# deryrahman/image-caption-emotion-indonesia

Hardware: AMD Instinct MI355X
Metric: images/sec (train step) + NLL loss match, batch=64 ResNet152+FactoredLSTM-512 (higher is better)
Workload: dtype f32 (trunk: operands as 2 f16 pieces each, 3 MFMA products per multiply, f32 accumulate; decoder: large products as 3 bf16 pieces per operand, 6 MFMA products per multiply, the rest f32 MFMA; the persistent LSTM kernel the trunk's split-f16 scheme)

## Files before the change

image-caption-emotion-indonesia_amd/csrc/fused_block.hip:

```cpp
#include <cstdlib>
#include <type_traits>

#include "common.h"
#include "mfma_core.h"
#include "split_f16.h"
#include "kernels.h"

namespace capnet {
namespace {

__host__ __device__ constexpr int fb_kslot(int g, int j) { return 16 * (j >> 2) + 4 * g + (j & 3); }


__global__ __launch_bounds__(256) void fb_pack_kernel(const float* __restrict__ w, unsigned* __restrict__ img, int C, int MID,
                                                      int role, int wide) {
  const int ew = f16x3_weight_shift(img[1]);
  if (blockIdx.x == 0 && threadIdx.x == 0) { img[0] = (unsigned)ew; img[2] = (unsigned)wide; }
  const float ws = ldexpf(1.f, ew);
  const long cells = (long)C * MID / 8 * 2;
  for (long i = (long)blockIdx.x * blockDim.x + threadIdx.x; i < cells; i += (long)gridDim.x * blockDim.x) {
    long r = i;
    const int lane = (int)(r & 63); r >>= 6;
    const int plane = (int)(r & 1); r >>= 1;
    const float* src;
// ... 30 lines not shown
      }
    }
    unsigned out[4];
#pragma unroll
    for (int q = 0; q < 4; ++q) {
      const float x0 = src[koff[2 * q]] * ws, x1 = src[koff[2 * q + 1]] * ws;
      _Float16 h0, l0, h1, l1;
      split1(x0, h0, l0);
      split1(x1, h1, l1);
      const h2 p = plane == 0 ? h2{h0, h1} : h2{l0, l1};
      out[q] = __builtin_bit_cast(unsigned, p);
    }
    unsigned* dst = img + kF16x3HdrWords + i * 4;
    dst[0] = out[0]; dst[1] = out[1]; dst[2] = out[2]; dst[3] = out[3];
  }
  if (role == 0) {
    float* cp = reinterpret_cast<float*>(img + kF16x3HdrWords + (long)C * MID);
    for (long i = (long)blockIdx.x * blockDim.x + threadIdx.x; i < (long)C * MID; i += (long)gridDim.x * blockDim.x) {
      const int c = (int)(i / MID), k = (int)(i - (long)c * MID);
      cp[((long)(c >> 4) * MID + k) * 16 + (c & 15)] = w[i];
    }
  }
}

static inline int fb_gram_rows(int K) { return K == 64 ? 512 : 256; }

struct GArgs {
  const float* y2; const float* s2; const float* t2;
  float* gp;
  float* cs;
  int M, K, in_exp, slices, pairs, slice_rows;
};

template <int K>
__global__ __launch_bounds__(256) void fb_gram_kernel(const GArgs g) {
  constexpr int NBLK = K / 64, NPAIR = NBLK * (NBLK + 1) / 2;
  constexpr int SR = K == 64 ? 128 : 64, NRG = SR / 8;
  constexpr int NCQ = K / 4, NIT = NCQ * NRG / 256;
  constexpr int kPlane = NRG * K * 16;
  static_assert(NIT >= 1 && NCQ * NRG == NIT * 256, "staging items");
  __shared__ __attribute__((aligned(16))) unsigned char lds[2 * kPlane];
  const int tid = threadIdx.x, lane = tid & 63, wave = tid >> 6;
  const int wm = wave >> 1, wn = wave & 1, li = lane & 31, lh = lane >> 5;
  const int slice = blockIdx.x, row0 = slice * g.slice_rows;
  const int rows = min(g.slice_rows, g.M - row0);
  const int nst = (rows + SR - 1) / SR;
  const float iscale = ldexpf(1.f, g.in_exp);
  const int chq = tid % NCQ, rgb = tid / NCQ;
  const f32x4 sc = *reinterpret_cast<const f32x4*>(g.s2 + 4 * chq), sh = *reinterpret_cast<const f32x4*>(g.t2 + 4 * chq);
  f32x4 colsum = {0.f, 0.f, 0.f, 0.f};
  f32x16 acc[NPAIR];
#pragma unroll
  for (int p = 0; p < NPAIR; ++p)
#pragma unroll
    for (int r = 0; r < 16; ++r) acc[p][r] = 0.f;
  f32x4 v[NIT][8];
  auto fetch = [&](int st) __attribute__((always_inline)) {
#pragma unroll
    for (int q = 0; q < NIT; ++q)
#pragma unroll
      for (int e = 0; e < 8; ++e) {
        const int m = row0 + st * SR + (rgb + q * (256 / NCQ)) * 8 + e;
        v[q][e] = *reinterpret_cast<const f32x4*>(g.y2 + (long)min(m, g.M - 1) * K + 4 * chq);
      }
  };
  auto stage = [&](int st) __attribute__((always_inline)) {
#pragma unroll
    for (int q = 0; q < NIT; ++q) {
      const int rg = rgb + q * (256 / NCQ);
      f32x4 x[8];
#pragma unroll
      for (int e = 0; e < 8; ++e) {
        const bool ok = row0 + st * SR + rg * 8 + e < row0 + rows;
#pragma unroll
        for (int c = 0; c < 4; ++c) {
          const float t = fmaxf(fmaf(v[q][e][c], sc[c], sh[c]), 0.f) * iscale;
          x[e][c] = ok ? t : 0.f;
          colsum[c] += x[e][c];
        }
      }
#pragma unroll
      for (int c = 0; c < 4; ++c) {
        const f32x4 a = {x[0][c], x[1][c], x[2][c], x[3][c]}, b = {x[4][c], x[5][c], x[6][c], x[7][c]};
        h4 ha, la, hb, lb;
        split4(a, ha, la);
        split4(b, hb, lb);
        unsigned char* d = lds + (rg * K + 4 * chq + c) * 16;
        *reinterpret_cast<h8*>(d) = cat8(ha, hb);
        *reinterpret_cast<h8*>(d + kPlane) = cat8(la, lb);
      }
    }
  };
  auto mma = [&]() __attribute__((always_inline)) {
#pragma unroll 2
    for (int k = 0; k < NRG / 2; ++k) {
      const unsigned char* base = lds + ((2 * k + lh) * K + li) * 16;
      h8 ah[NBLK], al[NBLK], bh[NBLK], bl[NBLK];
#pragma unroll
      for (int b = 0; b < NBLK; ++b) {
        ah[b] = *reinterpret_cast<const h8*>(base + (b * 64 + wm * 32) * 16);
        al[b] = *reinterpret_cast<const h8*>(base + (b * 64 + wm * 32) * 16 + kPlane);
        bh[b] = *reinterpret_cast<const h8*>(base + (b * 64 + wn * 32) * 16);
        bl[b] = *reinterpret_cast<const h8*>(base + (b * 64 + wn * 32) * 16 + kPlane);
      }
      int p = 0;
#pragma unroll
      for (int bi = 0; bi < NBLK; ++bi)
#pragma unroll
        for (int bj = bi; bj < NBLK; ++bj, ++p) {
          acc[p] = __builtin_amdgcn_mfma_f32_32x32x16_f16(al[bi], bh[bj], acc[p], 0, 0, 0);
          acc[p] = __builtin_amdgcn_mfma_f32_32x32x16_f16(ah[bi], bl[bj], acc[p], 0, 0, 0);
          acc[p] = __builtin_amdgcn_mfma_f32_32x32x16_f16(ah[bi], bh[bj], acc[p], 0, 0, 0);
        }
    }
  };
  fetch(0);
  for (int st = 0; st < nst; ++st) {
    stage(st);
    __syncthreads();
    fetch(st + 1 < nst ? st + 1 : st);
    mma();
    __syncthreads();
  }
  const float osc = ldexpf(1.f, -2 * g.in_exp);
#pragma unroll
  for (int p = 0; p < NPAIR; ++p) {
#pragma unroll
    for (int r = 0; r < 16; ++r) {
      const int m = wm * 32 + (r & 3) + 8 * (r >> 2) + 4 * lh;
      g.gp[(((long)p * 64 + m) * g.slices + slice) * 64 + wn * 32 + li] = acc[p][r] * osc;
    }
  }
  f32x4* cs_sh = reinterpret_cast<f32x4*>(lds);
  cs_sh[tid] = colsum;
  __syncthreads();
  if (tid < NCQ) {
    f32x4 t = cs_sh[tid];
#pragma unroll
    for (int q = 1; q < 256 / NCQ; ++q) t += cs_sh[q * NCQ + tid];
    *reinterpret_cast<f32x4*>(g.cs + (long)slice * K + 4 * tid) = t * ldexpf(1.f, -g.in_exp);
  }
}

__global__ __launch_bounds__(256) void fb_gram_reduce_kernel(const float* __restrict__ gp, const float* __restrict__ cs, float* __restrict__ G,
                                                             float* __restrict__ mu, int K, int slices, int pairs) {
  __shared__ double sh[8][32][4];
  const int it = threadIdx.x & 31, part = threadIdx.x >> 5;
  const int item_wgs = pairs * 32;
  if ((int)blockIdx.x < item_wgs) {
    const int item = blockIdx.x * 32 + it;
    const int n4 = item & 15, m = (item >> 4) & 63, pair = item >> 10;
    const float* p = gp + ((long)(pair * 64 + m) * slices) * 64 + 4 * n4;
    double s[4] = {0.0, 0.0, 0.0, 0.0};
    for (int s0 = part; s0 < slices; s0 += 64) {
      f32x4 v[8];
#pragma unroll
      for (int u = 0; u < 8; ++u) {
        const int sl = s0 + 8 * u;
        v[u] = *reinterpret_cast<const f32x4*>(p + (long)(sl < slices ? sl : part) * 64);
      }
#pragma unroll
      for (int u = 0; u < 8; ++u)
#pragma unroll
        for (int i = 0; i < 4; ++i) s[i] += (s0 + 8 * u < slices) ? (double)v[u][i] : 0.0;
    }
#pragma unroll
    for (int i = 0; i < 4; ++i) sh[part][it][i] = s[i];
    __syncthreads();
    if (part == 0) {
#pragma unroll
      for (int q = 1; q < 8; ++q)
#pragma unroll
        for (int i = 0; i < 4; ++i) s[i] += sh[q][it][i];
// ... 631 lines not shown
bool fused_block_shape_ok(long M, int MID) {
  return (MID == 64 || MID == 128 || MID == 256) && M > 0 && M < (1l << 24) && M * 4 * MID * 4 < (1l << 32);
}

size_t fused_block_weight_words(int C, int MID, int role) {
  return (size_t)kF16x3HdrWords + (size_t)C * MID * (role == 0 ? 2 : 1);
}

static bool fb_wide(int MID) {
  const char* e = getenv("CAPNET_FB_WIDE");
  if (e && (e[0] == '0' || e[0] == '1')) return e[0] == '1';
  (void)MID;
  return false;
}

int fused_block_pack(const float* w, unsigned* img, int C, int MID, int role, hipStream_t stream) {
  CAPNET_REQUIRE(w && img && aligned16(img) && C == 4 * MID && (MID == 64 || MID == 128 || MID == 256) && (role == 0 || role == 1),
                 "fused_block_pack: bad argument (C=%d MID=%d role=%d)", C, MID, role);
  const long n = (long)C * MID;
  const int rh = f16x3_pack_header(w, img, n, stream);
  if (rh) return rh;
  hipLaunchKernelGGL(fb_pack_kernel, dim3((int)(cdiv(n / 4, 256) > 2048 ? 2048 : cdiv(n / 4, 256))), dim3(256), 0, stream, w, img, C, MID, role, fb_wide(MID) ? 1 : 0);
  CAPNET_LAUNCH_CHECK();
  return kOk;
}

int fused_block_gram_slices(long M, int K) { return cdiv(M, fb_gram_rows(K)); }
int fused_block_gram_pairs(int K) { const int nb = K / 64; return nb * (nb + 1) / 2; }
size_t fused_block_stats_floats(long M, int K) {
  const size_t s = fused_block_gram_slices(M, K), p = fused_block_gram_pairs(K);
  return s * p * 4096 + ((s * K + 3) / 4 * 4) + ((size_t)K * K + K) + 8;
}

int fused_block_stats(const float* y2, const float* s2, const float* t2, const unsigned* w3img, long M, int MID, int in_exp,
                      const float* gamma, const float* beta, float* running_mean, float* running_var, float momentum, float eps,
                      float* scale, float* shift, float* batch_mean, float* batch_var, float* work, int* err, hipStream_t stream) {
  CAPNET_REQUIRE(y2 && s2 && t2 && w3img && scale && shift && work && aligned16(work) && aligned16(y2) && fused_block_shape_ok(M, MID) &&
                     in_exp > -64 && in_exp < 64, "fused_block_stats: bad argument");
  const int K = MID, C = 4 * MID;
  GArgs a;
  a.y2 = y2; a.s2 = s2; a.t2 = t2; a.M = (int)M; a.K = K; a.in_exp = in_exp;
  a.slices = fused_block_gram_slices(M, K); a.pairs = fused_block_gram_pairs(K); a.slice_rows = fb_gram_rows(K);
  a.gp = work;
  a.cs = work + (size_t)a.slices * a.pairs * 4096;
  float* G = a.cs + ((size_t)a.slices * K + 3) / 4 * 4;
  float* mu = G + (size_t)K * K;
  if (K == 256) hipLaunchKernelGGL(fb_gram_kernel<256>, dim3(a.slices), dim3(256), 0, stream, a);
  else if (K == 128) hipLaunchKernelGGL(fb_gram_kernel<128>, dim3(a.slices), dim3(256), 0, stream, a);
  else hipLaunchKernelGGL(fb_gram_kernel<64>, dim3(a.slices), dim3(256), 0, stream, a);
  hipLaunchKernelGGL(fb_gram_reduce_kernel, dim3(a.pairs * 32 + K / 32), dim3(256), 0, stream, a.gp, a.cs, G, mu, K, a.slices, a.pairs);
  const double inv = 1.0 / (double)M, unbias = M > 1 ? (double)M / (double)(M - 1) : 1.0;
  const float* wcopy = reinterpret_cast<const float*>(w3img + kF16x3HdrWords + (size_t)C * MID);
  if (K == 256)
    hipLaunchKernelGGL(fb_quad_kernel<256>, dim3(cdiv(C, kQC)), dim3(K * 4), 0, stream, G, mu, wcopy, C, inv, unbias, gamma, beta,
                       running_mean, running_var, momentum, eps, scale, shift, batch_mean, batch_var, err);
  else if (K == 128)
    hipLaunchKernelGGL(fb_quad_kernel<128>, dim3(cdiv(C, kQC)), dim3(K * 4), 0, stream, G, mu, wcopy, C, inv, unbias, gamma, beta,
                       running_mean, running_var, momentum, eps, scale, shift, batch_mean, batch_var, err);
  else
    hipLaunchKernelGGL(fb_quad_kernel<64>, dim3(cdiv(C, kQC)), dim3(K * 4), 0, stream, G, mu, wcopy, C, inv, unbias, gamma, beta,
                       running_mean, running_var, momentum, eps, scale, shift, batch_mean, batch_var, err);
  CAPNET_LAUNCH_CHECK();
  return kOk;
}

static void fb_shape(int MID, int* rs, int* nw) {
  (void)MID;
  const char* e = getenv("CAPNET_FB_RS");
  const char* w = getenv("CAPNET_FB_NW");
  *nw = (w && w[0] == '4') ? 4 : 8;
  *rs = (e && (e[0] == '1' || e[0] == '2')) ? e[0] - '0' : (*nw == 8 ? 1 : 2);
  if (*nw == 8) *rs = 1;
}
int fused_block_tiles(long M, int MID) {
  if (fb_wide(MID)) return cdiv(M, 128);
  int rs, nw;
  fb_shape(MID, &rs, &nw);
  return cdiv(M, 16 * rs * nw);
}

int fused_block_forward(const float* y2, const float* s2, const float* t2, const unsigned* w3img, const float* s3, const float* t3,
                        const float* res, const float* sd, const float* td, float* out, const unsigned* w1img, float* y1,
// ... 40 lines not shown
```

image-caption-emotion-indonesia_amd/_lib.py:

```python
import ctypes as C
import os

_HERE = os.path.dirname(os.path.abspath(__file__))
LIB_PATH = os.path.join(_HERE, "libcapnet_hip.so")

_f = C.POINTER(C.c_float)
_vp = C.c_void_p
_i = C.c_int
_l = C.c_long
_sz = C.c_size_t
_ip = C.POINTER(C.c_int)

SIGNATURES = {
    "capnet_last_error": (C.c_char_p, []),
    "capnet_abi_version": (_i, []),
    "capnet_sgemm": (_i, [_i, _i, _i, _i, _i, _vp, _l, _vp, _l, _vp, _l, _vp, _i, _i, _l, _l, _l,
                          _l, _i, _vp]),
    "capnet_sgemm_b3": (_i, [_i, _i, _i, _i, _i, _vp, _l, _vp, _l, _vp, _l, _vp, _i, _i, _l, _l, _l, _l, _vp, _sz, _vp]),
    "capnet_sgemm_b3_eligible": (_i, [_i, _i, _i, _i, _i, _vp, _l, _vp, _l, _vp, _l, _vp, _i, _l, _l, _l, _l]),
    "capnet_sgemm_splitk": (_i, [_i, _i, _i, _i, _i, _vp, _l, _vp, _l, _vp, _l, _vp, _i, _vp, _sz, _vp]),
    "capnet_sgemm_splitk_fused": (_i, [_i, _i, _i, _i, _i, _vp, _l, _vp, _l, _vp, _l, _vp, _i, _vp, _sz, _vp, _sz, _vp]),
    "capnet_colsum": (_i, [_vp, _l, _i, _i, _vp, _i, _vp]),
    "capnet_argmax_rows": (_i, [_vp, _i, _i, _i, _vp, _vp]),
    "capnet_resize_u8": (_i, [_vp, _i, _i, _vp, _vp, _i, _i, _vp, _vp, _i, _vp, _vp, _i, _vp]),
# ... 134 lines not shown
                                                                                                  _i, _vp, _vp, C.POINTER(_i),
                                                                                                  _vp, _vp]),
    "capnet_lstm_wfrag_floats": (_sz, [_i]),
    "capnet_lstm_pack_wfrag": (_i, [_vp, _vp, _i, _i, _vp]),
    "capnet_lstm_step_fused": (_i, [_vp, _vp, _vp, _l, _vp, _vp, _vp, _i, _i, _i, _vp]),
    "capnet_lstm_step_fused_stamped": (_i, [_vp, _vp, _vp, _l, _vp, _vp, _vp, _i, _i, _vp, _vp]),
    "capnet_lstm_step_fused_supported": (_i, [_i, _i]),
    "capnet_lstm_persist_supported": (_i, [_i, _i]),
    "capnet_lstm_persist_w_floats": (_sz, []),
    "capnet_lstm_persist_ctl_ints": (_sz, []),
    "capnet_lstm_persist_pack": (_i, [_vp, _vp, _i, _vp]),
    "capnet_lstm_persist_run": (_i, [_vp, _vp, _vp, _vp, _ip, _i, _i, _i, _i, _i, _vp, _vp, _vp, _vp]),
    "capnet_xent_fwd": (_i, [_vp, _l, _i, _i, _vp, _vp, _vp, _vp, _vp, _vp]),
    "capnet_xent_bwd": (_i, [_vp, _l, _i, _i, _vp, _vp, _vp, _vp, _l, _vp]),
    "capnet_att_loss_fwd": (_i, [_vp, _vp, _i, _i, _i, C.c_float, _vp, _vp, _vp]),
    "capnet_att_loss_bwd": (_i, [_vp, _vp, _i, _i, _i, C.c_float, _vp, _vp]),
    "capnet_clamp_adam": (_i, [_i, C.POINTER(_vp), C.POINTER(_vp), C.POINTER(_vp),
                               C.POINTER(_vp), C.POINTER(_l), _ip, C.c_float, C.c_float,
                               C.c_float, C.c_float, C.c_float, _i, _vp, _vp]),
    "capnet_lstm_persist_set_mode": (_i, [_i]),
    "capnet_att_set_chain_mode": (_i, [_i]),
    "capnet_lstm_pointwise_bwd": (_i, [_vp, _vp, _vp, _vp, _vp, _vp, _i, _i, _i, _vp]),
    "capnet_conv1x1_fwd_areg": (_i, [_vp, _vp, _i, _vp, _vp, _vp, _i, _vp, _vp, _l, _i, _i, _i, _vp]),
    "capnet_trunk_set_timing": (_i, [_vp, _i]),
    "capnet_trunk_time_next_pass": (_i, [_vp]),
    "capnet_trunk_collect_timing": (_i, [_vp, C.POINTER(C.c_double), C.POINTER(_l),
                                         C.POINTER(C.c_double)]),
    "capnet_packed_targets": (_i, [_vp, _i, _i, _ip, _vp, _vp]),
    "capnet_fused_block_weight_words": (_sz, [_i, _i, _i]),
    "capnet_fused_block_pack": (_i, [_vp, _vp, _i, _i, _i, _vp]),
    "capnet_fused_block_stats_floats": (_sz, [_l, _i]),
    "capnet_fused_block_stats": (_i, [_vp, _vp, _vp, _vp, _l, _i, _i, _vp, _vp, _vp, _vp, C.c_float, C.c_float, _vp, _vp, _vp,
                                      _vp, _vp]),
    "capnet_fused_block_tiles": (_i, [_l, _i]),
    "capnet_fused_block_forward": (_i, [_vp] * 14 + [_l, _i, _i, _i, _vp, _vp]),
    "capnet_comm_unique_id": (_i, [_vp]),
    "capnet_comm_create": (_i, [_vp, _i, _i, C.POINTER(_vp)]),
    "capnet_comm_destroy": (_i, [_vp]),
    "capnet_allreduce_grads": (_i, [_vp, _vp, _l, _vp]),
    "capnet_err_word_exchange": (_i, [_vp, _vp, _i, _vp]),
    "capnet_count_skipped": (_i, [_vp, _vp, _vp]),
    "capnet_pack_tensors": (_i, [_i, C.POINTER(_vp), C.POINTER(_l), _vp, _i, C.c_float, _vp]),
    "capnet_clamp": (_i, [_vp, _l, C.c_float, C.c_float, _vp]),
}


class CapnetError(RuntimeError):
    pass


_lib = None


def lib():
    global _lib
    if _lib is None:
        if not os.path.exists(LIB_PATH):
            raise CapnetError(
                "libcapnet_hip.so is not built (%s). Run `python -c 'import __graft_entry__ as g; "
                "g.build()'` or `make -C image-caption-emotion-indonesia_amd/csrc`. There is no "
                "CPU fallback." % LIB_PATH)
        l = C.CDLL(LIB_PATH)
        for name, (res, args) in SIGNATURES.items():
            fn = getattr(l, name)
            fn.restype = res
            fn.argtypes = args
# ... 32 lines not shown
```

image-caption-emotion-indonesia_amd/csrc/capi.cpp:

```cpp
#include "../../include/capnet.h"

#include "common.h"
#include "kernels.h"

using namespace capnet;

static inline hipStream_t S(capnet_stream_t s) { return reinterpret_cast<hipStream_t>(s); }

static SeqDims to_dims(const int* d) {
  SeqDims r;
  r.B = d[0]; r.T = d[1]; r.steps = d[2]; r.N = d[3]; r.E = d[4]; r.F = d[5]; r.H = d[6];
  r.V = d[7]; r.has_features = d[8]; r.cell = d[9];
  return r;
}

static bool weight_used(int cell, int i) { return cell == kCellFactored || i == 0 || i == 4 || i == 24 || i == 28; }
template <class Weights>
static void to_weights(const float* const* weights, Weights& w) {
  for (int g = 0; g < 4; ++g) {
    w.Vw[g] = weights[0 + g];  w.Vb[g] = weights[4 + g];
    w.Sw[g] = weights[8 + g];  w.Sb[g] = weights[12 + g];
    w.Uw[g] = weights[16 + g]; w.Ub[g] = weights[20 + g];
    w.Ww[g] = weights[24 + g]; w.Wb[g] = weights[28 + g];
  }
// ... 820 lines not shown
}

int capnet_packed_targets(const long long* captions, int T, int steps, const int* batch_sizes,
                          long long* out, capnet_stream_t stream) {
  CAPNET_REQUIRE(batch_sizes && steps > 0 && steps <= kMaxSteps, "packed_targets: steps %d", steps);
  SeqMeta m;
  m.steps = steps; m.has_features = 0; m.off[0] = 0;
  for (int t = 0; t < steps; ++t) {
    CAPNET_REQUIRE(batch_sizes[t] > 0, "packed_targets: batch_sizes[%d]", t);
    m.off[t + 1] = m.off[t] + batch_sizes[t];
    m.tf[t] = 1;
  }
  m.N = m.off[steps];
  return packed_targets(m, captions, T, out, S(stream));
}

int capnet_pack_tensors(int n, float* const* tensors, const long* numel, float* flat,
                        int direction, float scale, capnet_stream_t stream) {
  return pack_tensors(n, tensors, numel, flat, direction, scale, S(stream));
}

size_t capnet_fused_block_weight_words(int C, int MID, int role) { return fused_block_weight_words(C, MID, role); }
int capnet_fused_block_pack(const float* w, unsigned* img, int C, int MID, int role, capnet_stream_t stream) {
  return fused_block_pack(w, img, C, MID, role, S(stream));
}
size_t capnet_fused_block_stats_floats(long M, int MID) { return fused_block_stats_floats(M, MID); }
int capnet_fused_block_stats(const float* y2, const float* s2, const float* t2, const unsigned* w3img, long M, int MID,
                             int in_exp, const float* gamma, const float* beta, float* running_mean, float* running_var,
                             float momentum, float eps, float* scale, float* shift, float* work, int* err_flag,
                             capnet_stream_t stream) {
  return fused_block_stats(y2, s2, t2, w3img, M, MID, in_exp, gamma, beta, running_mean, running_var, momentum, eps, scale,
                           shift, nullptr, nullptr, work, err_flag, S(stream));
}
int capnet_fused_block_tiles(long M, int MID) { return fused_block_tiles(M, MID); }
int capnet_fused_block_forward(const float* y2, const float* s2, const float* t2, const unsigned* w3img, const float* s3,
                               const float* t3, const float* res, const float* sd, const float* td, float* out,
                               const unsigned* w1img, float* y1, float* part_sum, float* part_sq, long M, int MID, int e3,
                               int e1, int* err_flag, capnet_stream_t stream) {
  return fused_block_forward(y2, s2, t2, w3img, s3, t3, res, sd, td, out, w1img, y1, part_sum, part_sq, M, MID, e3, e1,
                             err_flag, S(stream));
}

int capnet_comm_unique_id(void* id128) { return comm_unique_id(id128); }
int capnet_comm_create(const void* id128, int rank, int world, capnet_comm_t** out) {
  return comm_create(id128, rank, world, reinterpret_cast<Comm**>(out));
}
int capnet_comm_destroy(capnet_comm_t* comm) { return comm_destroy(reinterpret_cast<Comm*>(comm)); }
int capnet_allreduce_grads(capnet_comm_t* comm, float* flat, long count, capnet_stream_t stream) {
  return allreduce_grads(reinterpret_cast<Comm*>(comm), flat, count, S(stream));
}

int capnet_err_word_exchange(int* err_flag, float* slot, int direction, capnet_stream_t stream) {
  return err_word_exchange(err_flag, slot, direction, S(stream));
}

int capnet_count_skipped(const int* err_flag, int* counter, capnet_stream_t stream) {
  return count_skipped(err_flag, counter, S(stream));
}

int capnet_clamp(float* x, long n, float lo, float hi, capnet_stream_t stream) {
  return clamp_inplace(x, n, lo, hi, S(stream));
}

}
```

image-caption-emotion-indonesia_amd/csrc/kernels.h:

```cpp
#pragma once
#include <hip/hip_runtime.h>

namespace capnet {

int sgemm(bool ta, bool tb, int M, int N, int K, const float* A, long lda, const float* B,
          long ldb, float* C, long ldc, const float* bias, int accumulate, int batch, long sA,
          long sB, long sC, long sBias, int force_tile, hipStream_t stream);

bool sgemm_b3_eligible(bool ta, bool tb, int M, int N, int K, const float* A, long lda, const float* B, long ldb,
                       const float* C, long ldc, const float* bias, int batch, long sA, long sB, long sC, long sBias);
int sgemm_b3(bool ta, bool tb, int M, int N, int K, const float* A, long lda, const float* B, long ldb, float* C, long ldc,
             const float* bias, int accumulate, int batch, long sA, long sB, long sC, long sBias, hipStream_t stream,
             float* ws = nullptr, size_t ws_floats = 0);

constexpr size_t kSplitKCounters = 1024;
int sgemm_splitk(bool ta, bool tb, int M, int N, int K, const float* A, long lda, const float* B,
                 long ldb, float* C, long ldc, const float* bias, int accumulate, float* ws,
                 size_t ws_floats, hipStream_t stream, int* counters = nullptr, size_t n_counters = 0);
int sgemm_splitk_slabs(bool tb, int M, int N, int K, const float* A, long lda, const float* B, long ldb,
                       float* ws, size_t ws_floats, int* n_slabs, hipStream_t stream);
int sgemm_rows16_slabs(bool tb, int M, int N, int K, const float* A, long lda, const float* B, long ldb, float* ws,
                       size_t ws_floats, int* n_slabs, hipStream_t stream);
int sgemm_splitk_batched(bool ta, bool tb, int M, int N, int K, const float* A, long lda,
                         const float* B, long ldb, float* C, long ldc, const float* bias,
// ... 250 lines not shown
                 float* datt2, long ldz, float* de_out, float* dwf_rows, float* dbf_rows,
                 hipStream_t stream, const float* dxa_slabs = nullptr, int n_slabs = 0, int emb_cols = 0);
int att_datt1(const float* att1, const float* att2_rows, long ldz2, const float* de_rows,
              const float* wf, const int* off, int steps, int B, int P, int A, float* datt1,
              hipStream_t stream);

int resize_u8(const unsigned char* src, int Hs, int Ws, unsigned char* tmp, unsigned char* dst, int Ho,
              int Wo, const int* bounds_h, const int* coef_h, int kmax_h, const int* bounds_v,
              const int* coef_v, int kmax_v, hipStream_t stream);
int crop_flip_normalize(const unsigned char* src, int B, int Hs, int Ws, const int* params, float* dst,
                        int Hc, int Wc, const float* mean, const float* stdv, hipStream_t stream);

int xent_fwd(const float* logits, long ld, int N, int V, const long long* targets, float* lse,
             float* row_loss, float* loss, int* err_flag, hipStream_t stream);
int topk_correct(const float* logits, long ld, int N, int V, const long long* targets, int k,
                 int* count, int* err_flag, hipStream_t stream);
int xent_bwd(const float* logits, long ld, int N, int V, const long long* targets,
             const float* lse, const float* gout, float* dlogits, long ldd, hipStream_t stream);
int att_loss_fwd(const float* nll, const float* alphas, int B, int steps, int P, float alpha_c,
                 float* colsum, float* out, hipStream_t stream);
int att_loss_bwd(const float* gout, const float* colsum, int B, int steps, int P, float alpha_c,
                 float* dalphas, hipStream_t stream);
int lstm_persist_set_mode(int mode);
int clamp_adam(int n_tensors, float* const* params, float* const* grads, float* const* exp_avg,
               float* const* exp_avg_sq, const long* numel, const int* step, float lr, float b1,
               float b2, float eps, float clip, int write_grad, const int* skip_flag, hipStream_t stream);
bool fused_block_shape_ok(long M, int MID);
size_t fused_block_weight_words(int C, int MID, int role);
int fused_block_pack(const float* w, unsigned* img, int C, int MID, int role, hipStream_t stream);
size_t fused_block_stats_floats(long M, int K);
int fused_block_stats(const float* y2, const float* s2, const float* t2, const unsigned* w3img, long M, int MID, int in_exp,
                      const float* gamma, const float* beta, float* running_mean, float* running_var, float momentum, float eps,
                      float* scale, float* shift, float* batch_mean, float* batch_var, float* work, int* err, hipStream_t stream);
int fused_block_tiles(long M, int MID);
int fused_block_forward(const float* y2, const float* s2, const float* t2, const unsigned* w3img, const float* s3, const float* t3,
                        const float* res, const float* sd, const float* td, float* out, const unsigned* w1img, float* y1,
                        float* part_sum, float* part_sq, long M, int MID, int e3, int e1, int* err, hipStream_t stream);
struct Comm;
int comm_unique_id(void* id128);
int comm_create(const void* id128, int rank, int world, Comm** out);
int comm_destroy(Comm* c);
int allreduce_grads(Comm* c, float* flat, long count, hipStream_t stream);
int err_word_exchange(int* err_flag, float* slot, int dir, hipStream_t stream);
int count_skipped(const int* err_flag, int* counter, hipStream_t stream);
int pack_tensors(int n_tensors, float* const* tensors, const long* numel, float* flat, int dir,
                 float scale, hipStream_t stream);
int clamp_inplace(float* x, long n, float lo, float hi, hipStream_t stream);
int bn1d_fwd(const float* x, int B, int C, const float* gamma, const float* beta, float* rmean,
             float* rvar, int train, float momentum, float eps, float* y, float* save_mean,
             float* save_invstd, hipStream_t stream);
int bn1d_bwd(const float* dy, const float* x, int B, int C, const float* gamma,
             const float* save_mean, const float* save_invstd, float* dx, float* dgamma,
             float* dbeta, hipStream_t stream);

constexpr int kCellFactored = 0;
constexpr int kCellLSTM = 1;
constexpr int kSeqInputDropoutOnly = 2;
struct SeqDims {
  int B, T, steps, N, E, F, H, V, has_features, cell;
};
struct SeqWeights {
  const float* Vw[4]; const float* Vb[4];
  const float* Sw[4]; const float* Sb[4];
  const float* Uw[4]; const float* Ub[4];
  const float* Ww[4]; const float* Wb[4];
};
// ... 69 lines not shown
```

include/capnet.h:

```cpp
#ifndef CAPNET_H_
#define CAPNET_H_

#include <stddef.h>

#ifdef __cplusplus
extern "C" {
#endif

typedef void* capnet_stream_t;
typedef struct capnet_trunk capnet_trunk_t;

#define CAPNET_OK 0
#define CAPNET_ERR_INVALID_ARG (-1)
#define CAPNET_ERR_HIP (-2)

const char* capnet_last_error(void);
int capnet_abi_version(void);

int capnet_sgemm(int transA, int transB, int M, int N, int K, const float* A, long lda,
                 const float* B, long ldb, float* C, long ldc, const float* bias, int accumulate,
                 int batch, long strideA, long strideB, long strideC, long strideBias,
                 int force_tile, capnet_stream_t stream);
int capnet_sgemm_b3(int transA, int transB, int M, int N, int K, const float* A, long lda, const float* B, long ldb,
                    float* C, long ldc, const float* bias, int accumulate, int batch, long strideA, long strideB,
// ... 330 lines not shown
int capnet_att_loss_fwd(const float* nll, const float* alphas, int B, int steps, int P, float alpha_c,
                        float* colsum, float* out, capnet_stream_t stream);
int capnet_att_loss_bwd(const float* gout, const float* colsum, int B, int steps, int P, float alpha_c,
                        float* dalphas, capnet_stream_t stream);

int capnet_resize_u8(const unsigned char* src, int Hs, int Ws, unsigned char* tmp, unsigned char* dst,
                     int Ho, int Wo, const int* bounds_h, const int* coef_h, int kmax_h,
                     const int* bounds_v, const int* coef_v, int kmax_v, capnet_stream_t stream);
int capnet_crop_flip_normalize(const unsigned char* src, int B, int Hs, int Ws, const int* params,
                               float* dst, int Hc, int Wc, const float* mean, const float* stdv,
                               capnet_stream_t stream);

int capnet_topk_correct(const float* logits, long ld, int N, int V, const long long* targets, int k,
                        int* count, int* err_flag, capnet_stream_t stream);

int capnet_clamp_adam(int n, float* const* params, float* const* grads, float* const* exp_avg,
                      float* const* exp_avg_sq, const long* numel, const int* step, float lr,
                      float beta1, float beta2, float eps, float clip, int write_grad,
                      const int* skip_flag, capnet_stream_t stream);

int capnet_packed_targets(const long long* captions, int T, int steps, const int* batch_sizes,
                          long long* out, capnet_stream_t stream);

int capnet_pack_tensors(int n, float* const* tensors, const long* numel, float* flat,
                        int direction, float scale, capnet_stream_t stream);

size_t capnet_fused_block_weight_words(int C, int MID, int role);
int capnet_fused_block_pack(const float* w, unsigned* img, int C, int MID, int role, capnet_stream_t stream);
size_t capnet_fused_block_stats_floats(long M, int MID);
int capnet_fused_block_stats(const float* y2, const float* s2, const float* t2, const unsigned* w3img, long M, int MID,
                             int in_exp, const float* gamma, const float* beta, float* running_mean, float* running_var,
                             float momentum, float eps, float* scale, float* shift, float* work, int* err_flag,
                             capnet_stream_t stream);
int capnet_fused_block_tiles(long M, int MID);
int capnet_fused_block_forward(const float* y2, const float* s2, const float* t2, const unsigned* w3img, const float* s3,
                               const float* t3, const float* res, const float* sd, const float* td, float* out,
                               const unsigned* w1img, float* y1, float* part_sum, float* part_sq, long M, int MID, int e3,
                               int e1, int* err_flag, capnet_stream_t stream);

typedef struct capnet_comm capnet_comm_t;
int capnet_comm_unique_id(void* id128);
int capnet_comm_create(const void* id128, int rank, int world, capnet_comm_t** out);
int capnet_comm_destroy(capnet_comm_t* comm);
int capnet_allreduce_grads(capnet_comm_t* comm, float* flat, long count, capnet_stream_t stream);

int capnet_err_word_exchange(int* err_flag, float* slot, int direction, capnet_stream_t stream);

int capnet_count_skipped(const int* err_flag, int* counter, capnet_stream_t stream);

int capnet_clamp(float* x, long n, float lo, float hi, capnet_stream_t stream);

#ifdef __cplusplus
}
#endif
#endif
```

Baseline: 9044.

## Restructure Gram kernel into 512-thread, two-half, double-buffered pipeline

The Gram statistics kernel moves from 256 to 512 threads. Two wave groups each own half of the block-pair accumulators, so register pressure per wave drops. LDS is double-buffered so staging of the next row tile overlaps the MFMA on the current one, and LDS fragment reads are software-pipelined with sched barriers. Channel cells get an XOR swizzle to reduce bank conflicts, and the ragged-row mask is applied only on the last tile. This costs twice the LDS and a more complex schedule, and it risks occupancy loss or mismatched writes if the half/slot mapping is wrong.

```diff
diff --git a/image-caption-emotion-indonesia_amd/csrc/fused_block.hip b/image-caption-emotion-indonesia_amd/csrc/fused_block.hip
--- a/image-caption-emotion-indonesia_amd/csrc/fused_block.hip
+++ b/image-caption-emotion-indonesia_amd/csrc/fused_block.hip
@@ -86,113 +86,163 @@
   int M, K, in_exp, slices, pairs, slice_rows;
 };
 
+__device__ __forceinline__ int fb_gram_cell(int ch) { return ch ^ ((ch >> 3) & 1); }
+__host__ __device__ constexpr int fb_gram_half(int nblk, int bi, int bj) { return nblk == 4 ? (bi == 1 || bi == 2) : (bi != bj); }
+__host__ __device__ constexpr int fb_gram_slot(int nblk, int bi, int bj) {
+  int n = 0;
+  for (int i = 0; i < nblk; ++i)
+    for (int j = i; j < nblk; ++j) {
+      if (i == bi && j == bj) return n;
+      if (fb_gram_half(nblk, i, j) == fb_gram_half(nblk, bi, bj)) ++n;
+    }
+  return n;
+}
+
 template <int K>
-__global__ __launch_bounds__(256) void fb_gram_kernel(const GArgs g) {
-  constexpr int NBLK = K / 64, NPAIR = NBLK * (NBLK + 1) / 2;
+__global__ __launch_bounds__(512) void fb_gram_kernel(const GArgs g) {
+  constexpr int NBLK = K / 64, NPAIR = NBLK * (NBLK + 1) / 2, NACC = (NPAIR + 1) / 2;
   constexpr int SR = K == 64 ? 128 : 64, NRG = SR / 8;
-  constexpr int NCQ = K / 4, NIT = NCQ * NRG / 256;
-  constexpr int kPlane = NRG * K * 16;
-  static_assert(NIT >= 1 && NCQ * NRG == NIT * 256, "staging items");
-  __shared__ __attribute__((aligned(16))) unsigned char lds[2 * kPlane];
-  const int tid = threadIdx.x, lane = tid & 63, wave = tid >> 6;
-  const int wm = wave >> 1, wn = wave & 1, li = lane & 31, lh = lane >> 5;
+  constexpr int NCP = K / 2, NRL = 512 / NCP, NIT = NRG / NRL;
+  constexpr int kPlane = NRG * K * 16, kImage = 2 * kPlane;
+  static_assert(NIT >= 1 && NRL * NIT == NRG, "staging items");
+  __shared__ __attribute__((aligned(16))) unsigned char lds[2 * kImage];
+  const int tid = threadIdx.x, lane = tid & 63, wave = __builtin_amdgcn_readfirstlane(tid >> 6);
+  const int wm = (wave >> 1) & 1, wn = wave & 1, li = fb_gram_cell(lane & 31), lh = lane >> 5;
   const int slice = blockIdx.x, row0 = slice * g.slice_rows;
   const int rows = min(g.slice_rows, g.M - row0);
   const int nst = (rows + SR - 1) / SR;
+  const bool ragged = rows % SR != 0;
+  const int chp = tid % NCP, rgb = tid / NCP;
   const float iscale = ldexpf(1.f, g.in_exp);
-  const int chq = tid % NCQ, rgb = tid / NCQ;
-  const f32x4 sc = *reinterpret_cast<const f32x4*>(g.s2 + 4 * chq), sh = *reinterpret_cast<const f32x4*>(g.t2 + 4 * chq);
-  f32x4 colsum = {0.f, 0.f, 0.f, 0.f};
-  f32x16 acc[NPAIR];
-#pragma unroll
-  for (int p = 0; p < NPAIR; ++p)
+  const f2 sc = *reinterpret_cast<const f2*>(g.s2 + 2 * chp) * iscale, sh = *reinterpret_cast<const f2*>(g.t2 + 2 * chp) * iscale;
+  const int cell0 = fb_gram_cell(2 * chp), cell1 = fb_gram_cell(2 * chp + 1);
+  f2 colsum = {0.f, 0.f};
+  f32x16 acc[NACC];
+#pragma unroll
+  for (int p = 0; p < NACC; ++p)
 #pragma unroll
     for (int r = 0; r < 16; ++r) acc[p][r] = 0.f;
-  f32x4 v[NIT][8];
-  auto fetch = [&](int st) __attribute__((always_inline)) {
+  f2 v[NIT][8];
+  auto fetch = [&](int st, f2 (&d)[NIT][8]) __attribute__((always_inline)) {
 #pragma unroll
     for (int q = 0; q < NIT; ++q)
 #pragma unroll
       for (int e = 0; e < 8; ++e) {
-        const int m = row0 + st * SR + (rgb + q * (256 / NCQ)) * 8 + e;
-        v[q][e] = *reinterpret_cast<const f32x4*>(g.y2 + (long)min(m, g.M - 1) * K + 4 * chq);
-      }
-  };
-  auto stage = [&](int st) __attribute__((always_inline)) {
+        const int m = row0 + st * SR + (rgb + q * NRL) * 8 + e;
+        d[q][e] = *reinterpret_cast<const f2*>(g.y2 + (long)min(m, g.M - 1) * K + 2 * chp);
+      }
+  };
+  auto stage_as = [&](int st, unsigned char* img, auto mask_c) __attribute__((always_inline)) {
+    constexpr bool MASK = decltype(mask_c)::value;
 #pragma unroll
     for (int q = 0; q < NIT; ++q) {
-      const int rg = rgb + q * (256 / NCQ);
-      f32x4 x[8];
+      const int rg = rgb + q * NRL;
+      f2 x[8];
 #pragma unroll
       for (int e = 0; e < 8; ++e) {
-        const bool ok = row0 + st * SR + rg * 8 + e < row0 + rows;
-#pragma unroll
-        for (int c = 0; c < 4; ++c) {
-          const float t = fmaxf(fmaf(v[q][e][c], sc[c], sh[c]), 0.f) * iscale;
+        const bool ok = !MASK || st * SR + rg * 8 + e < rows;
+#pragma unroll
+        for (int c = 0; c < 2; ++c) {
+          const float t = fmaxf(fmaf(v[q][e][c], sc[c], sh[c]), 0.f);
           x[e][c] = ok ? t : 0.f;
           colsum[c] += x[e][c];
         }
       }
 #pragma unroll
-      for (int c = 0; c < 4; ++c) {
+      for (int c = 0; c < 2; ++c) {
         const f32x4 a = {x[0][c], x[1][c], x[2][c], x[3][c]}, b = {x[4][c], x[5][c], x[6][c], x[7][c]};
         h4 ha, la, hb, lb;
         split4(a, ha, la);
         split4(b, hb, lb);
-        unsigned char* d = lds + (rg * K + 4 * chq + c) * 16;
+        unsigned char* d = img + (rg * K + (c == 0 ? cell0 : cell1)) * 16;
         *reinterpret_cast<h8*>(d) = cat8(ha, hb);
         *reinterpret_cast<h8*>(d + kPlane) = cat8(la, lb);
       }
     }
   };
-  auto mma = [&]() __attribute__((always_inline)) {
-#pragma unroll 2
+  auto stage = [&](int st, unsigned char* img) __attribute__((always_inline)) {
+    if (ragged && st == nst - 1) stage_as(st, img, std::true_type{});
+    else stage_as(st, img, std::false_type{});
+  };
+  auto mma = [&](const unsigned char* img, auto half_c) __attribute__((always_inline)) {
+    constexpr int HALF = decltype(half_c)::value;
+    h8 ah[2][NBLK], al[2][NBLK], bh[2][NBLK], bl[2][NBLK];
+    auto read = [&](int k) __attribute__((always_inline)) {
+      const unsigned char* base = img + ((2 * k + lh) * K + li) * 16;
+#pragma unroll
+      for (int b = 0; b < NBLK; ++b) {
+        ah[k & 1][b] = *reinterpret_cast<const h8*>(base + (b * 64 + wm * 32) * 16);
+        al[k & 1][b] = *reinterpret_cast<const h8*>(base + (b * 64 + wm * 32) * 16 + kPlane);
+        bh[k & 1][b] = *reinterpret_cast<const h8*>(base + (b * 64 + wn * 32) * 16);
+        bl[k & 1][b] = *reinterpret_cast<const h8*>(base + (b * 64 + wn * 32) * 16 + kPlane);
+      }
+    };
+    read(0);
+#pragma unroll
     for (int k = 0; k < NRG / 2; ++k) {
-      const unsigned char* base = lds + ((2 * k + lh) * K + li) * 16;
-      h8 ah[NBLK], al[NBLK], bh[NBLK], bl[NBLK];
-#pragma unroll
-      for (int b = 0; b < NBLK; ++b) {
-        ah[b] = *reinterpret_cast<const h8*>(base + (b * 64 + wm * 32) * 16);
-        al[b] = *reinterpret_cast<const h8*>(base + (b * 64 + wm * 32) * 16 + kPlane);
-        bh[b] = *reinterpret_cast<const h8*>(base + (b * 64 + wn * 32) * 16);
-        bl[b] = *reinterpret_cast<const h8*>(base + (b * 64 + wn * 32) * 16 + kPlane);
-      }
-      int p = 0;
+      if (k + 1 < NRG / 2) read(k + 1);
+      __builtin_amdgcn_sched_barrier(0);
 #pragma unroll
       for (int bi = 0; bi < NBLK; ++bi)
 #pragma unroll
-        for (int bj = bi; bj < NBLK; ++bj, ++p) {
-          acc[p] = __builtin_amdgcn_mfma_f32_32x32x16_f16(al[bi], bh[bj], acc[p], 0, 0, 0);
-          acc[p] = __builtin_amdgcn_mfma_f32_32x32x16_f16(ah[bi], bl[bj], acc[p], 0, 0, 0);
-          acc[p] = __builtin_amdgcn_mfma_f32_32x32x16_f16(ah[bi], bh[bj], acc[p], 0, 0, 0);
-        }
-    }
-  };
-  fetch(0);
-  for (int st = 0; st < nst; ++st) {
-    stage(st);
+        for (int bj = bi; bj < NBLK; ++bj) {
+          if (fb_gram_half(NBLK, bi, bj) != HALF) continue;
+          const int q = fb_gram_slot(NBLK, bi, bj);
+          acc[q] = __builtin_amdgcn_mfma_f32_32x32x16_f16(al[k & 1][bi], bh[k & 1][bj], acc[q], 0, 0, 0);
+          acc[q] = __builtin_amdgcn_mfma_f32_32x32x16_f16(ah[k & 1][bi], bl[k & 1][bj], acc[q], 0, 0, 0);
+          acc[q] = __builtin_amdgcn_mfma_f32_32x32x16_f16(ah[k & 1][bi], bh[k & 1][bj], acc[q], 0, 0, 0);
+        }
+      __builtin_amdgcn_sched_barrier(0);
+    }
+  };
+  auto run = [&](auto half_c) __attribute__((always_inline)) {
+    constexpr int HALF = decltype(half_c)::value;
+    for (int st = 0; st < nst; ++st) {
+      const unsigned char* cur = lds + (st & 1) * kImage;
+      unsigned char* nxt = lds + ((st + 1) & 1) * kImage;
+      if (HALF == 1) mma(cur, half_c);
+      if (st + 1 < nst) {
+        stage(st + 1, nxt);
+        if (st + 2 < nst) fetch(st + 2, v);
+      }
+      if (HALF == 0) mma(cur, half_c);
+      __syncthreads();
+    }
+  };
+  {
+    f2 v1[NIT][8];
+    fetch(0, v);
+    fetch(nst > 1 ? 1 : 0, v1);
+    stage(0, lds);
+#pragma unroll
+    for (int q = 0; q < NIT; ++q)
+#pragma unroll
+      for (int e = 0; e < 8; ++e) v[q][e] = v1[q][e];
     __syncthreads();
-    fetch(st + 1 < nst ? st + 1 : st);
-    mma();
-    __syncthreads();
-  }
+  }
+  if (wave < 4) run(std::integral_constant<int, 0>{});
+  else run(std::integral_constant<int, 1>{});
   const float osc = ldexpf(1.f, -2 * g.in_exp);
-#pragma unroll
-  for (int p = 0; p < NPAIR; ++p) {
-#pragma unroll
-    for (int r = 0; r < 16; ++r) {
-      const int m = wm * 32 + (r & 3) + 8 * (r >> 2) + 4 * lh;
-      g.gp[(((long)p * 64 + m) * g.slices + slice) * 64 + wn * 32 + li] = acc[p][r] * osc;
-    }
-  }
-  f32x4* cs_sh = reinterpret_cast<f32x4*>(lds);
+  const int half = wave >> 2;
+  const long mstride = (long)g.slices * 64;
+  float* const out = g.gp + ((long)(wm * 32 + 4 * lh) * g.slices + slice) * 64 + wn * 32 + (lane & 31);
+  int p = 0;
+#pragma unroll
+  for (int bi = 0; bi < NBLK; ++bi)
+#pragma unroll
+    for (int bj = bi; bj < NBLK; ++bj, ++p) {
+      if (fb_gram_half(NBLK, bi, bj) != half) continue;
+#pragma unroll
+      for (int r = 0; r < 16; ++r) out[(p * 64 + (r & 3) + 8 * (r >> 2)) * mstride] = acc[fb_gram_slot(NBLK, bi, bj)][r] * osc;
+    }
+  f2* cs_sh = reinterpret_cast<f2*>(lds);
   cs_sh[tid] = colsum;
   __syncthreads();
-  if (tid < NCQ) {
-    f32x4 t = cs_sh[tid];
-#pragma unroll
-    for (int q = 1; q < 256 / NCQ; ++q) t += cs_sh[q * NCQ + tid];
-    *reinterpret_cast<f32x4*>(g.cs + (long)slice * K + 4 * tid) = t * ldexpf(1.f, -g.in_exp);
+  if (tid < NCP) {
+    f2 t = cs_sh[tid];
+#pragma unroll
+    for (int q = 1; q < NRL; ++q) t += cs_sh[q * NCP + tid];
+    *reinterpret_cast<f2*>(g.cs + (long)slice * K + 2 * tid) = t * ldexpf(1.f, -g.in_exp);
   }
 }
 
@@ -903,9 +953,9 @@
   a.cs = work + (size_t)a.slices * a.pairs * 4096;
   float* G = a.cs + ((size_t)a.slices * K + 3) / 4 * 4;
   float* mu = G + (size_t)K * K;
-  if (K == 256) hipLaunchKernelGGL(fb_gram_kernel<256>, dim3(a.slices), dim3(256), 0, stream, a);
-  else if (K == 128) hipLaunchKernelGGL(fb_gram_kernel<128>, dim3(a.slices), dim3(256), 0, stream, a);
-  else hipLaunchKernelGGL(fb_gram_kernel<64>, dim3(a.slices), dim3(256), 0, stream, a);
+  if (K == 256) hipLaunchKernelGGL(fb_gram_kernel<256>, dim3(a.slices), dim3(512), 0, stream, a);
+  else if (K == 128) hipLaunchKernelGGL(fb_gram_kernel<128>, dim3(a.slices), dim3(512), 0, stream, a);
+  else hipLaunchKernelGGL(fb_gram_kernel<64>, dim3(a.slices), dim3(512), 0, stream, a);
   hipLaunchKernelGGL(fb_gram_reduce_kernel, dim3(a.pairs * 32 + K / 32), dim3(256), 0, stream, a.gp, a.cs, G, mu, K, a.slices, a.pairs);
   const double inv = 1.0 / (double)M, unbias = M > 1 ? (double)M / (double)(M - 1) : 1.0;
   const float* wcopy = reinterpret_cast<const float*>(w3img + kF16x3HdrWords + (size_t)C * MID);
```

Result: no change. 9022 (-0.2%).

## Add 512-thread warp-specialized Gram kernel for K=256 fused block stats

Applied to the files above, without the earlier changes.

Adds a new Gram-matrix kernel for the K=256 fused-block batch-norm statistics. It uses 512 threads: waves 0-3 stage the normalized, ReLU'd input into double-buffered LDS as split-f16 planes while also computing one block row. Waves 4-7 compute the remaining upper-triangular 64x64 blocks with 32x32x16 MFMAs. The LDS layout is swizzled to avoid bank conflicts. The aim is to overlap global loads and staging with the matrix work and to cover the symmetric Gram with more waves. It becomes the default, and a runtime switch keeps the old kernel selectable. The new kernel uses more LDS and registers and splits work unevenly between the two wave groups.

```diff
diff --git a/image-caption-emotion-indonesia_amd/_lib.py b/image-caption-emotion-indonesia_amd/_lib.py
--- a/image-caption-emotion-indonesia_amd/_lib.py
+++ b/image-caption-emotion-indonesia_amd/_lib.py
@@ -190,6 +190,7 @@
     "capnet_fused_block_stats_floats": (_sz, [_l, _i]),
     "capnet_fused_block_stats": (_i, [_vp, _vp, _vp, _vp, _l, _i, _i, _vp, _vp, _vp, _vp, C.c_float, C.c_float, _vp, _vp, _vp,
                                       _vp, _vp]),
+    "capnet_fused_block_set_stats_variant": (_i, [_i]),
     "capnet_fused_block_tiles": (_i, [_l, _i]),
     "capnet_fused_block_forward": (_i, [_vp] * 14 + [_l, _i, _i, _i, _vp, _vp]),
     "capnet_comm_unique_id": (_i, [_vp]),
diff --git a/image-caption-emotion-indonesia_amd/csrc/capi.cpp b/image-caption-emotion-indonesia_amd/csrc/capi.cpp
--- a/image-caption-emotion-indonesia_amd/csrc/capi.cpp
+++ b/image-caption-emotion-indonesia_amd/csrc/capi.cpp
@@ -876,6 +876,7 @@
   return fused_block_stats(y2, s2, t2, w3img, M, MID, in_exp, gamma, beta, running_mean, running_var, momentum, eps, scale,
                            shift, nullptr, nullptr, work, err_flag, S(stream));
 }
+int capnet_fused_block_set_stats_variant(int variant) { return fused_block_set_stats_variant(variant); }
 int capnet_fused_block_tiles(long M, int MID) { return fused_block_tiles(M, MID); }
 int capnet_fused_block_forward(const float* y2, const float* s2, const float* t2, const unsigned* w3img, const float* s3,
                                const float* t3, const float* res, const float* sd, const float* td, float* out,
diff --git a/image-caption-emotion-indonesia_amd/csrc/fused_block.hip b/image-caption-emotion-indonesia_amd/csrc/fused_block.hip
--- a/image-caption-emotion-indonesia_amd/csrc/fused_block.hip
+++ b/image-caption-emotion-indonesia_amd/csrc/fused_block.hip
@@ -187,6 +187,130 @@
   }
   f32x4* cs_sh = reinterpret_cast<f32x4*>(lds);
   cs_sh[tid] = colsum;
+  __syncthreads();
+  if (tid < NCQ) {
+    f32x4 t = cs_sh[tid];
+#pragma unroll
+    for (int q = 1; q < 256 / NCQ; ++q) t += cs_sh[q * NCQ + tid];
+    *reinterpret_cast<f32x4*>(g.cs + (long)slice * K + 4 * tid) = t * ldexpf(1.f, -g.in_exp);
+  }
+}
+
+__device__ __forceinline__ int fb_gram_swz(int ch) { return ch ^ ((ch >> 3) & 3); }
+
+template <int BI0, int BI1>
+__device__ __forceinline__ void fb_gram8_mma(const unsigned char* __restrict__ img, int kplane, int cell, int wm, int wn, int lh,
+                                            f32x16 (&acc)[6]) {
+  constexpr int K = 256, NBLK = 4;
+#pragma unroll
+  for (int k = 0; k < 2; ++k) {
+    const unsigned char* base = img + ((2 * k + lh) * K + cell) * 16;
+    h8 bh[NBLK], bl[NBLK];
+#pragma unroll
+    for (int b = BI0; b < NBLK; ++b) {
+      bh[b] = *reinterpret_cast<const h8*>(base + (b * 64 + wn * 32) * 16);
+      bl[b] = *reinterpret_cast<const h8*>(base + (b * 64 + wn * 32) * 16 + kplane);
+    }
+    int p = 0;
+#pragma unroll
+    for (int bi = BI0; bi < BI1; ++bi) {
+      const h8 ah = *reinterpret_cast<const h8*>(base + (bi * 64 + wm * 32) * 16);
+      const h8 al = *reinterpret_cast<const h8*>(base + (bi * 64 + wm * 32) * 16 + kplane);
+#pragma unroll
+      for (int bj = bi; bj < NBLK; ++bj, ++p) {
+        acc[p] = __builtin_amdgcn_mfma_f32_32x32x16_f16(al, bh[bj], acc[p], 0, 0, 0);
+        acc[p] = __builtin_amdgcn_mfma_f32_32x32x16_f16(ah, bl[bj], acc[p], 0, 0, 0);
+        acc[p] = __builtin_amdgcn_mfma_f32_32x32x16_f16(ah, bh[bj], acc[p], 0, 0, 0);
+      }
+    }
+  }
+}
+
+__global__ __launch_bounds__(512, 2) void fb_gram8_kernel(const GArgs g) {
+  constexpr int K = 256, NCQ = K / 4;
+  constexpr int HR = 32, NRG = HR / 8;
+  constexpr int kPlane = NRG * K * 16, kImg = 2 * kPlane;
+  static_assert(NCQ * NRG == 256, "one staging item per thread of waves 0-3 and half step");
+  __shared__ __attribute__((aligned(16))) unsigned char lds[2 * kImg];
+  const int tid = threadIdx.x, lane = tid & 63, wave = tid >> 6, grp = wave >> 2;
+  const int wm = (wave >> 1) & 1, wn = wave & 1, li = lane & 31, lh = lane >> 5;
+  const int slice = blockIdx.x, row0 = slice * g.slice_rows;
+  const int rows = min(g.slice_rows, g.M - row0);
+  const int nh = 2 * ((rows + 2 * HR - 1) / (2 * HR));
+  const float iscale = ldexpf(1.f, g.in_exp);
+  const int chq = tid & (NCQ - 1), rg = (tid >> 6) & (NRG - 1);
+  const f32x4 sc = *reinterpret_cast<const f32x4*>(g.s2 + 4 * chq), sh = *reinterpret_cast<const f32x4*>(g.t2 + 4 * chq);
+  f32x4 colsum = {0.f, 0.f, 0.f, 0.f};
+  f32x16 acc[6];
+#pragma unroll
+  for (int p = 0; p < 6; ++p)
+#pragma unroll
+    for (int r = 0; r < 16; ++r) acc[p][r] = 0.f;
+  f32x4 v[8];
+  auto fetch = [&](int h) __attribute__((always_inline)) {
+#pragma unroll
+    for (int e = 0; e < 8; ++e) {
+      const int m = row0 + h * HR + rg * 8 + e;
+      v[e] = *reinterpret_cast<const f32x4*>(g.y2 + (long)min(m, g.M - 1) * K + 4 * chq);
+    }
+  };
+  auto stage = [&](int h) __attribute__((always_inline)) {
+    f32x4 x[8];
+#pragma unroll
+    for (int e = 0; e < 8; ++e) {
+      const bool ok = row0 + h * HR + rg * 8 + e < row0 + rows;
+#pragma unroll
+      for (int c = 0; c < 4; ++c) {
+        const float t = fmaxf(fmaf(v[e][c], sc[c], sh[c]), 0.f) * iscale;
+        x[e][c] = ok ? t : 0.f;
+        colsum[c] += x[e][c];
+      }
+    }
+    unsigned char* img = lds + (h & 1) * kImg + rg * K * 16;
+#pragma unroll
+    for (int c = 0; c < 4; ++c) {
+      const f32x4 a = {x[0][c], x[1][c], x[2][c], x[3][c]}, b = {x[4][c], x[5][c], x[6][c], x[7][c]};
+      h4 ha, la, hb, lb;
+      split4(a, ha, la);
+      split4(b, hb, lb);
+      unsigned char* d = img + fb_gram_swz(4 * chq + c) * 16;
+      *reinterpret_cast<h8*>(d) = cat8(ha, hb);
+      *reinterpret_cast<h8*>(d + kPlane) = cat8(la, lb);
+    }
+  };
+  const int cell = fb_gram_swz(li);
+  if (grp == 0) {
+    fetch(0);
+    stage(0);
+    fetch(nh > 1 ? 1 : 0);
+  }
+  __syncthreads();
+  for (int h = 0; h < nh; ++h) {
+    const unsigned char* img = lds + (h & 1) * kImg;
+    if (grp == 0) {
+      if (h + 1 < nh) {
+        stage(h + 1);
+        fetch(h + 2 < nh ? h + 2 : h + 1);
+      }
+      fb_gram8_mma<0, 1>(img, kPlane, cell, wm, wn, lh, acc);
+    } else {
+      fb_gram8_mma<1, 4>(img, kPlane, cell, wm, wn, lh, acc);
+    }
+    __syncthreads();
+  }
+  const float osc = ldexpf(1.f, -2 * g.in_exp);
+#pragma unroll
+  for (int j = 0; j < 6; ++j) {
+    if (grp == 0 && j >= 4) break;
+    const int p = grp == 0 ? j : 4 + j;
+#pragma unroll
+    for (int r = 0; r < 16; ++r) {
+      const int m = wm * 32 + (r & 3) + 8 * (r >> 2) + 4 * lh;
+      g.gp[(((long)p * 64 + m) * g.slices + slice) * 64 + wn * 32 + li] = acc[j][r] * osc;
+    }
+  }
+  f32x4* cs_sh = reinterpret_cast<f32x4*>(lds);
+  if (grp == 0) cs_sh[tid] = colsum;
   __syncthreads();
   if (tid < NCQ) {
     f32x4 t = cs_sh[tid];
@@ -890,6 +1014,13 @@
   return s * p * 4096 + ((s * K + 3) / 4 * 4) + ((size_t)K * K + K) + 8;
 }
 
+static int g_fb_stats_variant = 0;
+int fused_block_set_stats_variant(int variant) {
+  const int old = g_fb_stats_variant;
+  g_fb_stats_variant = variant ? 1 : 0;
+  return old;
+}
+
 int fused_block_stats(const float* y2, const float* s2, const float* t2, const unsigned* w3img, long M, int MID, int in_exp,
                       const float* gamma, const float* beta, float* running_mean, float* running_var, float momentum, float eps,
                       float* scale, float* shift, float* batch_mean, float* batch_var, float* work, int* err, hipStream_t stream) {
@@ -903,7 +1034,8 @@
   a.cs = work + (size_t)a.slices * a.pairs * 4096;
   float* G = a.cs + ((size_t)a.slices * K + 3) / 4 * 4;
   float* mu = G + (size_t)K * K;
-  if (K == 256) hipLaunchKernelGGL(fb_gram_kernel<256>, dim3(a.slices), dim3(256), 0, stream, a);
+  if (K == 256 && g_fb_stats_variant == 0) hipLaunchKernelGGL(fb_gram8_kernel, dim3(a.slices), dim3(512), 0, stream, a);
+  else if (K == 256) hipLaunchKernelGGL(fb_gram_kernel<256>, dim3(a.slices), dim3(256), 0, stream, a);
   else if (K == 128) hipLaunchKernelGGL(fb_gram_kernel<128>, dim3(a.slices), dim3(256), 0, stream, a);
   else hipLaunchKernelGGL(fb_gram_kernel<64>, dim3(a.slices), dim3(256), 0, stream, a);
   hipLaunchKernelGGL(fb_gram_reduce_kernel, dim3(a.pairs * 32 + K / 32), dim3(256), 0, stream, a.gp, a.cs, G, mu, K, a.slices, a.pairs);
diff --git a/image-caption-emotion-indonesia_amd/csrc/kernels.h b/image-caption-emotion-indonesia_amd/csrc/kernels.h
--- a/image-caption-emotion-indonesia_amd/csrc/kernels.h
+++ b/image-caption-emotion-indonesia_amd/csrc/kernels.h
@@ -306,6 +306,7 @@
 int fused_block_stats(const float* y2, const float* s2, const float* t2, const unsigned* w3img, long M, int MID, int in_exp,
                       const float* gamma, const float* beta, float* running_mean, float* running_var, float momentum, float eps,
                       float* scale, float* shift, float* batch_mean, float* batch_var, float* work, int* err, hipStream_t stream);
+int fused_block_set_stats_variant(int variant);
 int fused_block_tiles(long M, int MID);
 int fused_block_forward(const float* y2, const float* s2, const float* t2, const unsigned* w3img, const float* s3, const float* t3,
                         const float* res, const float* sd, const float* td, float* out, const unsigned* w1img, float* y1,
diff --git a/include/capnet.h b/include/capnet.h
--- a/include/capnet.h
+++ b/include/capnet.h
@@ -386,6 +386,7 @@
                              int in_exp, const float* gamma, const float* beta, float* running_mean, float* running_var,
                              float momentum, float eps, float* scale, float* shift, float* work, int* err_flag,
                              capnet_stream_t stream);
+int capnet_fused_block_set_stats_variant(int variant);
 int capnet_fused_block_tiles(long M, int MID);
 int capnet_fused_block_forward(const float* y2, const float* s2, const float* t2, const unsigned* w3img, const float* s3,
                                const float* t3, const float* res, const float* sd, const float* td, float* out,
```

New measurement: 8877 before, 8961 after (median of 6 runs). No clear change (+0.9%).
